# omarkhursheed/whisper-sae

Hardware: AMD Instinct MI355X
Metric: activations/sec through SAE train step (d=384->3072, k=32) (higher is better)
Workload: dtype bf16; 1 GPU; BASELINE.json configs[1]: TopKSAE 384->3072 k=32 train step, synthetic activations resident in the HBM ring buffer; batch_per_gpu=16384, global_batch=16384, ring_rows_per_gpu=4194304, parallelism=dp1

## Files before the change

include/wsae.h:

```cpp
#ifndef WSAE_H_
#define WSAE_H_

#include <stddef.h>
#include <stdint.h>

#ifdef __cplusplus
extern "C" {
#endif

#define WSAE_VERSION 1

#define WSAE_OK 0
#define WSAE_ERR_INVALID (-1)
#define WSAE_ERR_HIP (-2)
#define WSAE_ERR_NOMEM (-3)

#define WSAE_PREC_BF16 0
#define WSAE_PREC_FP32 1

#define WSAE_DT_F32 0
#define WSAE_DT_BF16 1

typedef struct wsae_ctx wsae_ctx;
typedef struct wsae_ring wsae_ring;

typedef struct wsae_config {
    int32_t input_dim;
    int32_t hidden_dim;
    int32_t k;
    int32_t max_batch;
    int32_t precision;
    int32_t device;
} wsae_config;

typedef struct wsae_stats {
    float loss;
    float l0;
    float grad_norm;
    float clip_coef;
    float dead_ratio;
    int32_t dead_count;
    int32_t topk_fallback_rows;
    int32_t reserved;
} wsae_stats;

const char* wsae_last_error(void);
int wsae_version(void);

int64_t wsae_param_count(int32_t input_dim, int32_t hidden_dim);
int wsae_param_offsets(int32_t input_dim, int32_t hidden_dim, int64_t offsets[5]);

int wsae_ctx_create(const wsae_config* cfg, wsae_ctx** out);
int wsae_ctx_destroy(wsae_ctx* ctx);
int wsae_ctx_set_fired(wsae_ctx* ctx, float* fired);
int wsae_ctx_set_strip_predict(wsae_ctx* ctx, int32_t on, float assume_store_threshold);
int wsae_ctx_strip_stats(wsae_ctx* ctx, int64_t* refilled_rows, float* last_min_threshold, float* margin);
int wsae_ctx_set_loss_cols(wsae_ctx* ctx, int32_t cols);
size_t wsae_ctx_workspace_bytes(const wsae_ctx* ctx);
int wsae_ctx_reserve_relu(wsae_ctx* ctx);

int wsae_prepare(wsae_ctx* ctx, const float* params, void* stream);


int wsae_encode_topk(wsae_ctx* ctx, const float* params, const void* x, int32_t x_dtype,
                     const int32_t* rows, int32_t B, float* vals, int32_t* idx,
                     int64_t* step_count, wsae_stats* stats, void* stream);

int wsae_encode_dense(wsae_ctx* ctx, const float* params, const void* x, int32_t x_dtype,
                      const int32_t* rows, int32_t B, float* pre, void* stream);

int wsae_densify(wsae_ctx* ctx, const float* vals, const int32_t* idx, int32_t B, float* hidden,
                 void* stream);

int wsae_decode_dense(wsae_ctx* ctx, const float* params, const float* hidden, int32_t B,
                      float* recon, void* stream);

int wsae_decode_loss(wsae_ctx* ctx, const float* params, const void* x, int32_t x_dtype,
                     const int32_t* rows, const float* vals, const int32_t* idx, int32_t B,
                     float* recon, int32_t want_bwd, float* dpre, int64_t* last_activated,
                     const int64_t* step_count, wsae_stats* stats, void* stream);

int wsae_encode_decode(wsae_ctx* ctx, const float* params, const void* x, int32_t x_dtype, const int32_t* rows,
                       int32_t B, float* vals, int32_t* idx, int64_t* step_count, float* recon, int32_t want_bwd,
                       float* dpre, int64_t* last_activated, wsae_stats* stats, void* stream);

int wsae_weight_grads(wsae_ctx* ctx, const float* params, const void* x, int32_t x_dtype,
                      const int32_t* rows, const float* vals, const int32_t* idx,
                      const float* dpre, int32_t B, float* grads, void* stream);

#define WSAE_BTK_TRAIN 0
#define WSAE_BTK_EVAL 1
#define WSAE_BTK_SELECT 2
typedef struct wsae_batch_topk_state {
    float threshold;
    float beta;
    float last_t;
    int32_t saturated_rows;
    int32_t kept;
    int32_t reserved[3];
} wsae_batch_topk_state;
int wsae_batch_topk_select(wsae_ctx* ctx, float* vals, int32_t B, int32_t k_batch, int32_t mode,
                           wsae_batch_topk_state* state, void* stream);
int wsae_ctx_set_batch_topk(wsae_ctx* ctx, int32_t k_batch, int32_t mode, wsae_batch_topk_state* state);

#define WSAE_PART_ALL (-1)
#define WSAE_PART_DECODER 0
#define WSAE_PART_ENCODER 1
int wsae_wgrad_parts_supported(const wsae_ctx* ctx);
int wsae_ctx_set_comm_reserve(wsae_ctx* ctx, int32_t n_cus);
int wsae_weight_grads_wire(wsae_ctx* ctx, const float* params, const void* x, int32_t x_dtype,
                           const int32_t* rows, const float* vals, const int32_t* idx, const float* dpre,
                           int32_t B, int32_t part, void* wire, int32_t wire_dtype, void* stream);

int wsae_last_residual_grad(wsae_ctx* ctx, int32_t B, float* g_out, void* stream);

int wsae_input_grad(wsae_ctx* ctx, const float* params, const int32_t* idx, const float* dpre,
                    int32_t B, float* dx, int32_t subtract_g, void* stream);

#define WSAE_WIRE_METRIC_SLOTS 24
int wsae_ctx_set_wire_metrics(wsae_ctx* ctx, const float* loss_l0);
int wsae_grads_unpack_wire(wsae_ctx* ctx, const void* wire, int32_t wire_dtype, float* grads_ext,
                           const float* metrics_sum, int32_t world, wsae_stats* stats, void* stream);
int wsae_adamw_step(wsae_ctx* ctx, float* params, const float* grads, float* exp_avg,
                    float* exp_avg_sq, float lr, float beta1, float beta2, float eps,
                    float weight_decay, int32_t step, float max_norm, float grad_scale,
                    int32_t normalize_decoder, int32_t norm_from_wgrad,
                    int64_t* last_activated, const int64_t* step_count,
                    int64_t dead_threshold, wsae_stats* stats, void* stream);

int wsae_normalize_decoder(wsae_ctx* ctx, float* params, void* stream);

int wsae_dead_scan(wsae_ctx* ctx, const int64_t* last_activated, const int64_t* step_count,
                   int64_t threshold, uint8_t* mask, wsae_stats* stats, void* stream);

int wsae_row_errors(wsae_ctx* ctx, const void* x, int32_t x_dtype, const int32_t* rows,
                    const float* recon, int32_t B, float* row_err, float* resid, void* stream);
int wsae_resample_dead(wsae_ctx* ctx, float* params, const void* inputs, int32_t x_dtype,
                       const int32_t* rows, int32_t Br, const float* row_err,
                       const uint8_t* dead_mask, int64_t* last_activated,
                       const int64_t* step_count, int32_t num_cap, int32_t* n_dead_out,
                       const float* dec_src, void* stream);

int wsae_ring_create(int32_t device, int64_t capacity_rows, int32_t dim, int32_t dtype,
                     wsae_ring** out);
int wsae_ring_destroy(wsae_ring* ring);
int wsae_ring_push_layernorm(wsae_ring* ring, const void* src, int32_t src_dtype, int64_t n_rows,
                             const float* gamma, const float* beta, float eps, void* stream);
void* wsae_ring_data(wsae_ring* ring);
int64_t wsae_ring_size(const wsae_ring* ring);
int wsae_ring_push(wsae_ring* ring, const void* src, int32_t src_dtype, int64_t n_rows, void* stream);
int wsae_ring_sample(wsae_ring* ring, uint64_t seed, int64_t epoch, int64_t offset, int32_t n,
                     int32_t* rows_out, void* stream);
int wsae_ring_fill_synthetic(wsae_ring* ring, uint64_t seed, int64_t n_rows, void* stream);

#define WSAE_IV_KEEP_ERROR 0
#define WSAE_IV_REPLACE 1
#define WSAE_IV_MAX_FORCE 64
int wsae_layernorm_rows(const void* src, int32_t src_dtype, int64_t n_rows, int32_t dim, const float* gamma,
                        const float* beta, float eps, void* dst, int32_t dst_dtype, void* stream);
int wsae_intervene(wsae_ctx* ctx, const float* params, const void* h, int32_t h_dtype, int64_t n_rows,
                   const float* vals, const int32_t* idx, const float* gamma, const float* beta, float eps,
                   const float* scale, const int32_t* force_idx, const float* force_val, int32_t n_force,
                   const uint8_t* row_mask, int32_t mode, void* out, int32_t out_dtype, int32_t* changed_rows,
                   void* stream);

#define WSAE_K_STAGE_BATCH 0
#define WSAE_K_ENCODE_GEMM 1
#define WSAE_K_TOPK 2
#define WSAE_K_DECODE 3
#define WSAE_K_BUCKET 4
#define WSAE_K_WGRAD 5
#define WSAE_K_WGRAD_REDUCE 6
#define WSAE_K_SQNORM 7
#define WSAE_K_ADAMW 8
#define WSAE_K_ROWNORM 9
#define WSAE_K_PREPARE 10
#define WSAE_K_DEAD_SCAN 11
#define WSAE_K_COUNT 12
const char* wsae_kernel_name(int32_t kernel_id);
int wsae_profile_enable(wsae_ctx* ctx, int32_t kernel_id, int32_t max_samples);
int wsae_profile_disable(wsae_ctx* ctx);
int wsae_profile_read(wsae_ctx* ctx, int32_t kernel_id, int32_t* n_launches, double* total_ms);

int64_t wsae_feature_topk_workspace_bytes(int64_t max_entries, int32_t H);
int wsae_feature_topk_update(const float* vals, const int32_t* idx, int64_t rows, int32_t width, int32_t H,
                             int32_t keep, int64_t ord_base, float* top_vals, int64_t* top_ord,
                             int32_t* top_cnt, int64_t* total_active, void* workspace,
                             int64_t workspace_bytes, void* stream);

int wsae_ctx_set_relu_fp8(wsae_ctx* ctx, int32_t on);
int wsae_relu_needs_hidden(const wsae_ctx* ctx, int32_t B);
int wsae_ctx_set_relu_l1_weights(wsae_ctx* ctx, const float* weights);
int wsae_relu_forward(wsae_ctx* ctx, const float* params, const void* x, int32_t x_dtype,
                      const int32_t* rows, int32_t B, float sparsity_weight, float* hidden,
                      float* recon, wsae_stats* stats, float* sparsity_loss_out, void* stream);
int wsae_relu_backward(wsae_ctx* ctx, const float* params, const void* x, int32_t x_dtype,
                       const int32_t* rows, int32_t B, float sparsity_weight, const float* hidden,
                       const float* recon, float* grads, void* stream);

#ifdef __cplusplus
}
#endif
#endif
```

whisper-sae_amd/csrc/wsae_ctx.hip:

```cpp
#include <stdarg.h>
#include <stdlib.h>
#include <string.h>

#include <new>

#include "wsae_common.h"
#include "wsae_topk.h"
#include <cstdlib>
#include <vector>

static thread_local char g_err[512] = "";
static void prof_free(wsae_ctx* c);

void wsae_set_error(const char* fmt, ...) {
    va_list ap;
    va_start(ap, fmt);
    vsnprintf(g_err, sizeof(g_err), fmt, ap);
    va_end(ap);
}

extern "C" const char* wsae_last_error(void) { return g_err; }
extern "C" int wsae_version(void) { return WSAE_VERSION; }

extern "C" int64_t wsae_param_count(int32_t D, int32_t H) {
// ... 111 lines not shown
    c->WdT_bf16 = (bf16_t*)(base + o_wd);
    c->c_fold = (float*)(base + o_cf);
    c->xb = base + o_xb;
    c->xT = base + o_xT;
    c->gT = base + o_gT;
    c->g = (float*)(base + o_g);
    c->gb = (bf16_t*)(base + o_gb);
    c->pre = (float*)(base + o_pre);
    c->smax = (float*)(base + o_sm);
    c->part_loss = (float*)(base + o_pl);
    c->part_l0 = (float*)(base + o_p0);
    c->part_dbd = (float*)(base + o_pd);
    c->part_sq = (float*)(base + o_ps);
    c->dbd2 = (float*)(base + o_d2);
    c->colnorm = (float*)(base + o_cn);
    c->counters = (int32_t*)(base + o_ct);
    c->wg_slabs = (float*)(base + o_ws);
    c->dbe_slab = (float*)(base + o_ds);
    c->dbpre_part = (float*)(base + o_dp);
    c->ent_pos = (uint32_t*)(base + o_ep);
    c->ent_hid = base + o_eh;
    c->ent_dpre = base + o_ed;
    c->ent_off = (int32_t*)(base + o_eo);
    c->dead_list = (int32_t*)(base + o_dl);
    c->row_order = (int32_t*)(base + o_ro);
    c->tmin = (uint32_t*)(base + o_tm);
    c->btk_ws = (int32_t*)(base + o_bt);
    const char* sp = getenv("WSAE_STRIP_PREDICT");
    c->strip_predict = (sp && sp[0] == '0') ? 0 : 1;
    const char* ss = getenv("WSAE_STRIP_SAFETY");
    c->tg_fixed_s = ss ? (float)atof(ss) : 0.f;
    c->ws_bytes = cv.total;
    *out = c;
    return WSAE_OK;
}

extern "C" int wsae_ctx_destroy(wsae_ctx* ctx) {
    if (!ctx) return WSAE_OK;
    prof_free(ctx);
    if (ctx->relu_ws) (void)hipFree(ctx->relu_ws);
    if (ctx->We_bf16) (void)hipFree((void*)ctx->We_bf16);
    delete ctx;
    return WSAE_OK;
}

static const char* const k_names[WSAE_K_COUNT] = {"stage_batch", "encode_gemm", "topk", "decode", "bucket", "wgrad",
                                                  "wgrad_reduce", "sqnorm", "adamw", "rownorm", "prepare", "dead_scan"};

extern "C" const char* wsae_kernel_name(int32_t id) { return (id >= 0 && id < WSAE_K_COUNT) ? k_names[id] : "?"; }

static void prof_free(wsae_ctx* c) {
    for (int k = 0; k < WSAE_K_COUNT; ++k) {
        if (c->prof.ev[k]) {
            for (int i = 0; i < 2 * c->prof.max_samples; ++i) (void)hipEventDestroy(c->prof.ev[k][i]);
            delete[] c->prof.ev[k];
            c->prof.ev[k] = nullptr;
        }
        c->prof.count[k] = 0;
    }
    c->prof.mask = 0;
    c->prof.max_samples = 0;
}

extern "C" int wsae_profile_disable(wsae_ctx* ctx) {
    WSAE_REQUIRE(ctx, "wsae_profile_disable: null ctx");
    prof_free(ctx);
    return WSAE_OK;
}

extern "C" int wsae_profile_enable(wsae_ctx* ctx, int32_t kernel_id, int32_t max_samples) {
    WSAE_REQUIRE(ctx && kernel_id >= -1 && kernel_id < WSAE_K_COUNT && max_samples >= 1 && max_samples <= 65536,
                 "wsae_profile_enable: bad argument");
    prof_free(ctx);
    ctx->prof.max_samples = max_samples;
    for (int k = 0; k < WSAE_K_COUNT; ++k) {
        if (kernel_id != -1 && kernel_id != k) continue;
        ctx->prof.ev[k] = new (std::nothrow) hipEvent_t[2 * (size_t)max_samples];
        if (!ctx->prof.ev[k]) {
            wsae_set_error("out of host memory");
            return WSAE_ERR_NOMEM;
        }
        for (int i = 0; i < 2 * max_samples; ++i) WSAE_HIP_CHECK(hipEventCreate(&ctx->prof.ev[k][i]));
        ctx->prof.mask |= 1u << k;
    }
    return WSAE_OK;
}

extern "C" int wsae_profile_read(wsae_ctx* ctx, int32_t kernel_id, int32_t* n_launches, double* total_ms) {
    WSAE_REQUIRE(ctx && kernel_id >= 0 && kernel_id < WSAE_K_COUNT && n_launches && total_ms,
                 "wsae_profile_read: bad argument");
    *n_launches = 0;
    *total_ms = 0.0;
    if (!ctx->prof.ev[kernel_id]) return WSAE_OK;
    const int n = ctx->prof.count[kernel_id];
    double tot = 0.0;
    for (int i = 0; i < n; ++i) {
        WSAE_HIP_CHECK(hipEventSynchronize(ctx->prof.ev[kernel_id][2 * i + 1]));
        float ms = 0.f;
        WSAE_HIP_CHECK(hipEventElapsedTime(&ms, ctx->prof.ev[kernel_id][2 * i], ctx->prof.ev[kernel_id][2 * i + 1]));
        tot += ms;
    }
    *n_launches = n;
    *total_ms = tot;
    return WSAE_OK;
}

extern "C" int wsae_ctx_set_fired(wsae_ctx* ctx, float* fired) {
    WSAE_REQUIRE(ctx, "wsae_ctx_set_fired: null ctx");
    ctx->fired = fired;
    return WSAE_OK;
}

static uint32_t host_f32_ord(float f) {
    uint32_t u;
    memcpy(&u, &f, 4);
    return (u & 0x80000000u) ? ~u : (u | 0x80000000u);
}
extern "C" int wsae_ctx_set_strip_predict(wsae_ctx* ctx, int32_t on, float assume_store_threshold) {
    WSAE_REQUIRE(ctx, "wsae_ctx_set_strip_predict: null ctx");
    ctx->strip_predict = on ? 1 : 0;
    ctx->pred_valid = 0;
    WSAE_HIP_CHECK(hipDeviceSynchronize());
    const bool forget = assume_store_threshold != assume_store_threshold;
    const float one = 1.0f;
    uint32_t hdr[3] = {forget ? 0u : host_f32_ord(assume_store_threshold), 0u, 0u};
    if (!forget) memcpy(&hdr[1], &one, 4);
    uint32_t* prev = ctx->tmin + ctx->tmin_cur * TG_GROUP_WORDS;
    WSAE_HIP_CHECK(hipMemset(prev, 0, TG_GROUP_WORDS * 4));
    WSAE_HIP_CHECK(hipMemset(ctx->tmin + ((ctx->tmin_cur + 2) % 3) * TG_GROUP_WORDS, 0, TG_GROUP_WORDS * 4));
    WSAE_HIP_CHECK(hipMemcpy(prev, hdr, sizeof(hdr), hipMemcpyHostToDevice));
    return WSAE_OK;
}
extern "C" int wsae_ctx_strip_stats(wsae_ctx* ctx, int64_t* refilled_rows, float* last_min_threshold, float* margin) {
    WSAE_REQUIRE(ctx && refilled_rows && last_min_threshold && margin, "wsae_ctx_strip_stats: null argument");
    std::vector<uint32_t> h(TG_WORDS);
    WSAE_HIP_CHECK(hipDeviceSynchronize());
    WSAE_HIP_CHECK(hipMemcpy(h.data(), ctx->tmin, h.size() * 4, hipMemcpyDeviceToHost));
    *refilled_rows = (int64_t)h[TG_REFILLED];
    uint32_t o = 0xFFFFFFFFu;
    for (int i = 0; i < TG_SLOTS; ++i) {
        const uint32_t s = h[ctx->tmin_cur * TG_GROUP_WORDS + i * TG_SLOT_STRIDE];
        if (s != 0u && s < o) o = s;
    }
    float f = NAN;
    if (o != 0u && o != 0xFFFFFFFFu) {
        const uint32_t u = (o & 0x80000000u) ? (o & 0x7FFFFFFFu) : ~o;
        memcpy(&f, &u, 4);
    }
    *last_min_threshold = f;
    memcpy(margin, &h[ctx->tmin_cur * TG_GROUP_WORDS + TG_HDR_S], 4);
    return WSAE_OK;
}

extern "C" int wsae_ctx_set_wire_metrics(wsae_ctx* ctx, const float* loss_l0) {
    WSAE_REQUIRE(ctx, "wsae_ctx_set_wire_metrics: null ctx");
    ctx->wire_metrics = loss_l0;
    return WSAE_OK;
}

extern "C" int wsae_ctx_set_loss_cols(wsae_ctx* ctx, int32_t cols) {
    WSAE_REQUIRE(ctx && cols >= 1 && cols <= ctx->D, "wsae_ctx_set_loss_cols: columns must be in [1, input_dim]");
    ctx->loss_cols = cols;
    return WSAE_OK;
}

extern "C" size_t wsae_ctx_workspace_bytes(const wsae_ctx* ctx) { return ctx ? ctx->ws_bytes : 0; }

__global__ void __launch_bounds__(256) prepare_kernel(const float* __restrict__ We, const float* __restrict__ WdT,
                                                      const float* __restrict__ be, const float* __restrict__ bpre,
                                                      bf16_t* __restrict__ We16, bf16_t* __restrict__ WdT16,
                                                      float* __restrict__ cfold, int H, int D) {
    const int lane = threadIdx.x & 63;
    const int h = blockIdx.x * 4 + (threadIdx.x >> 6);
    if (h >= H) return;
    const float* row = We + (int64_t)h * D;
    bf16_t* orow = We16 + (int64_t)h * D;
    const float* drow = WdT + (int64_t)h * D;
    bf16_t* odrow = WdT16 + (int64_t)h * D;
    float dot = 0.f;
    for (int d = lane * 4; d < D; d += 256) {
        const float4 wd = *(const float4*)(drow + d);
        bf16x4 o, e;
        o[0] = (bf16_t)wd.x; o[1] = (bf16_t)wd.y; o[2] = (bf16_t)wd.z; o[3] = (bf16_t)wd.w;
        *(bf16x4*)(odrow + d) = o;
        const float4 w = *(const float4*)(row + d);
        e[0] = (bf16_t)w.x; e[1] = (bf16_t)w.y; e[2] = (bf16_t)w.z; e[3] = (bf16_t)w.w;
        *(bf16x4*)(orow + d) = e;
        const float4 bp = *(const float4*)(bpre + d);
        dot = fmaf((float)e[0], bp.x, dot);
        dot = fmaf((float)e[1], bp.y, dot);
        dot = fmaf((float)e[2], bp.z, dot);
        dot = fmaf((float)e[3], bp.w, dot);
    }
    dot = wave_sum(dot);
    if (lane == 0) cfold[h] = be[h] - dot;
}

int wsae_prepare_launch(wsae_ctx* ctx, const float* params, hipStream_t st) {
    if (ctx->prec != WSAE_PREC_BF16) return WSAE_OK;
    WSAE_PROF_BEGIN(ctx, WSAE_K_PREPARE, st);
    prepare_kernel<<<ceil_div(ctx->H, 4), 256, 0, st>>>(params + ctx->off[0], params + ctx->off[1],
                                                        params + ctx->off[2], params + ctx->off[4], ctx->We_bf16,
                                                        ctx->WdT_bf16, ctx->c_fold, ctx->H, ctx->D);
    WSAE_PROF_END(ctx, WSAE_K_PREPARE, st);
    WSAE_LAUNCH_CHECK();
    return WSAE_OK;
}

extern "C" int wsae_prepare(wsae_ctx* ctx, const float* params, void* stream) {
    WSAE_REQUIRE(ctx && params, "wsae_prepare: null argument");
    return wsae_prepare_launch(ctx, params, (hipStream_t)stream);
}
```

whisper-sae_amd/csrc/wsae_encode.hip:

```cpp
#include "wsae_common.h"
#include "wsae_mfma.h"
#include "wsae_topk.h"

template <typename T>
__device__ __forceinline__ void store4(T* p, const float (&v)[4]) {
    if (sizeof(T) == 2) {
        bf16x4 o;
#pragma unroll
        for (int i = 0; i < 4; ++i) o[i] = (bf16_t)v[i];
        *(bf16x4*)p = o;
    } else {
        *(float4*)p = make_float4(v[0], v[1], v[2], v[3]);
    }
}

template <int XDT>
__device__ __forceinline__ void load4(const void* x, int64_t i, float (&v)[4]) {
    if (XDT == WSAE_DT_BF16) {
        const bf16x4 t = *(const bf16x4*)((const bf16_t*)x + i);
#pragma unroll
        for (int q = 0; q < 4; ++q) v[q] = (float)t[q];
    } else {
        const float4 t = *(const float4*)((const float*)x + i);
        v[0] = t.x; v[1] = t.y; v[2] = t.z; v[3] = t.w;
    }
}

template <int XDT, typename T>
__global__ void __launch_bounds__(256) stage_batch_kernel(const void* __restrict__ x, const int32_t* __restrict__ rows,
                                                          const float* __restrict__ bpre, T* __restrict__ xb,
                                                          T* __restrict__ xT, int B, int D, int ldT,
                                                          int64_t* __restrict__ step_count) {
    __shared__ float tile[64][65];
    if (step_count && blockIdx.x == 0 && blockIdx.y == 0 && threadIdx.x == 0) *step_count += 1;
    const int b0 = blockIdx.x * 64, d0 = blockIdx.y * 64;
    const int q = threadIdx.x & 15, r16 = threadIdx.x >> 4;
#pragma unroll
    for (int p = 0; p < 4; ++p) {
        const int bl = r16 + 16 * p, b = b0 + bl, d = d0 + 4 * q;
        float v[4] = {0.f, 0.f, 0.f, 0.f};
        if (b < B && d < D) {
            const int64_t src = rows ? (int64_t)rows[b] : (int64_t)b;
            load4<XDT>(x, src * D + d, v);
            if (sizeof(T) == 4) {
                const float4 bp = *(const float4*)(bpre + d);
                v[0] -= bp.x; v[1] -= bp.y; v[2] -= bp.z; v[3] -= bp.w;
            }
            store4<T>(xb + (int64_t)b * D + d, v);
        }
#pragma unroll
        for (int i = 0; i < 4; ++i) tile[bl][4 * q + i] = v[i];
    }
    if (!xT) return;
    __syncthreads();
#pragma unroll
    for (int p = 0; p < 4; ++p) {
        const int dl = r16 + 16 * p, d = d0 + dl, b = b0 + 4 * q;
        if (d < D && b < ldT) {
            float v[4];
#pragma unroll
            for (int i = 0; i < 4; ++i) v[i] = (T)tile[4 * q + i][dl];
            store4<T>(xT + (int64_t)d * ldT + b, v);
        }
    }
}

__global__ void __launch_bounds__(256) stage_rows_copy_kernel(const uint4* __restrict__ x, const int32_t* __restrict__ rows,
                                                              uint4* __restrict__ xb, int64_t nchunks, int cpr,
                                                              int64_t* __restrict__ step_count) {
    if (step_count && blockIdx.x == 0 && threadIdx.x == 0) *step_count += 1;
    const int64_t i0 = (int64_t)blockIdx.x * 512 + threadIdx.x, i1 = i0 + 256;
    const int64_t j0 = min(i0, nchunks - 1), j1 = min(i1, nchunks - 1);
    const int b0 = (int)(j0 / cpr), b1 = (int)(j1 / cpr);
    const int64_t r0 = rows ? (int64_t)rows[b0] : (int64_t)b0, r1 = rows ? (int64_t)rows[b1] : (int64_t)b1;
    const uint4 v0 = x[r0 * cpr + (j0 - (int64_t)b0 * cpr)];
    const uint4 v1 = x[r1 * cpr + (j1 - (int64_t)b1 * cpr)];
    if (i0 < nchunks) xb[i0] = v0;
    if (i1 < nchunks) xb[i1] = v1;
}

#ifdef WSAE_ENC_STAMPS
__device__ unsigned long long enc_stamp_sum[8];
#define EN_T(i)                                                                                     \
    {                                                                                               \
        __builtin_amdgcn_sched_barrier(0);                                                          \
        unsigned long long t_;                                                                      \
        asm volatile("s_memtime %0\n\ts_waitcnt lgkmcnt(0)" : "=s"(t_)::"memory");                  \
        __builtin_amdgcn_sched_barrier(0);                                                          \
        en_acc[i] += t_ - en_last;                                                                  \
        en_last = t_;                                                                               \
    }
extern "C" int wsae_debug_enc_stamps(double* out, int reset) {
    unsigned long long h[8];
    if (hipMemcpyFromSymbol(h, HIP_SYMBOL(enc_stamp_sum), sizeof(h)) != hipSuccess) return -1;
    for (int i = 0; i < 8; ++i) out[i] = (double)h[i];
    if (reset) {
        unsigned long long z[8] = {0, 0, 0, 0, 0, 0, 0, 0};
        (void)hipMemcpyToSymbol(HIP_SYMBOL(enc_stamp_sum), z, sizeof(z));
    }
    return 0;
}
#else
#define EN_T(i)
#endif
#define G256D_STAGE (2 * 256 * SWZ_ROW_BYTES)
#define G256D_STAGE1 (72 * 1024)
#define G256D_LDS (G256D_STAGE1 + G256D_STAGE)

template <typename T>
__global__ void __launch_bounds__(512)
encode_gemm256d_kernel(const T* __restrict__ xb, int64_t lda, const T* __restrict__ W, int64_t ldb,
                       const float* __restrict__ bias, float* __restrict__ pre, int64_t ldp, int B, int H, int D, int ntn,
                       int ntiles_mn, int nsplit, int64_t cz, float* __restrict__ smax, const int32_t* __restrict__ arows,
                       int64_t* __restrict__ step_count, const float* __restrict__ rscale = nullptr,
                       const float* __restrict__ cscale = nullptr, uint32_t* __restrict__ tmin = nullptr, int tmin_cur = 0,
                       float tg_fixed_s = 0.f) {
    extern __shared__ __attribute__((aligned(16))) char smem[];
    constexpr int KT = SWZ_ROW_BYTES / (int)sizeof(T);
    constexpr int EPC = 16 / (int)sizeof(T);
    const int tid = threadIdx.x, lane = tid & 63, wave = tid >> 6;
    const int wm = wave >> 2, wn = wave & 3;
    const int nk = D / KT;
    const int col = lane & 31, rq = lane >> 5;
    constexpr int PS = 68;
    float* patch = (float*)smem + wave * 32 * PS;
    const int pr = lane >> 4, pc = (lane & 15) * 4;
    const uint32_t smem_lds = (uint32_t)(uintptr_t)(__attribute__((address_space(3))) char*)smem;
    const int dma_r = lane >> 3, dma_s = lane & 7;
    if (step_count && blockIdx.x == 0 && tid == 0) *step_count += 1;
    __shared__ float tg_sh;
    if (wave == 0) {
        float s_now = 0.f;
        const float t = tmin ? strip_store_threshold(tmin, tmin_cur, lane, tg_fixed_s, &s_now) : -INFINITY;
        if (lane == 0) tg_sh = t;
        if (tmin && blockIdx.x == 0) {
            uint32_t* grp = tmin + tmin_cur * TG_GROUP_WORDS;
            grp[lane * TG_SLOT_STRIDE] = 0xFFFFFFFFu;
            if (lane == 0) {
                grp[TG_HDR_S] = __float_as_uint(s_now);
                grp[TG_HDR_MISSES] = 0u;
                __builtin_nontemporal_store(t, (float*)tmin + TG_USED);
            }
        }
    }

    const int ntiles = ntiles_mn * nsplit;
    const int ntm = ntiles_mn / ntn;
    const bool xcd_walk = nsplit == 1 && (gridDim.x % 8 == 0) && (ntm % 8 == 0);
    const int xcd = blockIdx.x & 7, local = blockIdx.x >> 3, per_xcd = gridDim.x >> 3;
    auto tile_at = [&](int i) -> int {
        if (!xcd_walk) return (int)blockIdx.x + i * (int)gridDim.x;
        const int tl = local + i * per_xcd;
        if (tl >= (ntm >> 3) * ntn) return ntiles;
        return (xcd * (ntm >> 3) + tl / ntn) * ntn + tl % ntn;
    };
    auto a_rows = [&](int m0, int (&ar)[4]) {
#pragma unroll
        for (int j = 0; j < 4; ++j) {
            const int m = min(m0 + (wave + 8 * j) * 8 + dma_r, B - 1);
            ar[j] = arows ? arows[m] : m;
        }
    };
    auto dma = [&](const int (&ar)[4], int n0, int64_t k0, int st) {
        const uint32_t base = smem_lds + (st ? G256D_STAGE1 : 0);
#pragma unroll
        for (int j = 0; j < 8; ++j) {
            const int piece = wave + 8 * j;
            const int row = (piece & 31) * 8 + dma_r;
            const int c = dma_s ^ ((row >> 1) & 7);
            const T* src = j < 4 ? xb + (int64_t)ar[j & 3] * lda + k0 + c * EPC
                                 : W + (int64_t)min(n0 + row, H - 1) * ldb + k0 + c * EPC;
            glds16(src, base + piece * 1024);
        }
    };
    auto m_of = [&](int t) { return ((t % ntiles_mn) / ntn) * 256; };
    auto n_of = [&](int t) { return ((t % ntiles_mn) % ntn) * 256; };
    auto k_of = [&](int t) { return (int64_t)(t / ntiles_mn) * D; };

#ifdef WSAE_ENC_STAMPS
    unsigned long long en_acc[8] = {0, 0, 0, 0, 0, 0, 0, 0}, en_last = __builtin_amdgcn_s_memtime();
#endif
    int it = 0, st = 1;
    int tile = tile_at(0);
    int ar[4] = {0, 0, 0, 0}, ar_n[4];
    if (tile < ntiles) {
        a_rows(m_of(tile), ar);
        dma(ar, n_of(tile), k_of(tile), st);
    }
    for (; tile < ntiles; tile = tile_at(++it)) {
        const int m0 = m_of(tile), n0 = n_of(tile);
        const int64_t kbase = k_of(tile);
        const int z = tile / ntiles_mn;
        f32x16 acc[4][2];
#pragma unroll
        for (int i = 0; i < 4; ++i)
#pragma unroll
            for (int j = 0; j < 2; ++j)
#pragma unroll
                for (int r = 0; r < 16; ++r) acc[i][j][r] = 0.f;
        const int nt = min(tile_at(it + 1), ntiles - 1);
        a_rows(m_of(nt), ar_n);
        EN_T(0)
        for (int kt = 0; kt < nk; ++kt) {
            dma_wait();
            EN_T(1)
            __syncthreads();
            EN_T(2)
            if (kt + 1 < nk) dma(ar, n0, kbase + (int64_t)(kt + 1) * KT, st ^ 1);
            else dma(ar_n, n_of(nt), k_of(nt), st ^ 1);
            EN_T(3)
            const char* As = smem + (st ? G256D_STAGE1 : 0);
            Mfma256s<T>::slab(As, As + 256 * SWZ_ROW_BYTES, wm * 128, wn * 64, lane, acc);
            st ^= 1;
            EN_T(4)
        }
        __syncthreads();
        EN_T(5)
        const int hcol = n0 + wn * 64 + pc;
        float4 bv4 = make_float4(0.f, 0.f, 0.f, 0.f);
        if (bias && z == 0 && hcol < H) bv4 = *(const float4*)(bias + hcol);
        const float tg = tg_sh;
        const bool fast = !rscale && smax && z == 0 && m0 + 256 <= B && n0 + 256 <= H && (int64_t)B * ldp < (1ll << 29);
        if (fast) {
            typedef int i32x4 __attribute__((ext_vector_type(4)));
            const __amdgpu_buffer_rsrc_t r_pre = __builtin_amdgcn_make_buffer_rsrc(pre, 0, 0x7fffffff, 0x00020000);
            const __amdgpu_buffer_rsrc_t r_sm = __builtin_amdgcn_make_buffer_rsrc(smax, 0, 0x7fffffff, 0x00020000);
            const int hs = H >> 4;
            const int b_lane = m0 + wm * 128 + pr;
            const int off_pre = (int)(((int64_t)b_lane * ldp + hcol) * 4);
            const int off_sm = (b_lane * hs + (hcol >> 4)) * 4;
            const int row_pre = (int)ldp * 16, row_sm = hs * 16;
#pragma unroll
            for (int mi = 0; mi < 4; ++mi) {
#pragma unroll
                for (int ni = 0; ni < 2; ++ni)
#pragma unroll
                    for (int r = 0; r < 16; ++r)
                        patch[((r & 3) + 8 * (r >> 2) + 4 * rq) * PS + ni * 32 + col] = acc[mi][ni][r];
                __builtin_amdgcn_wave_barrier();
                EN_T(6)
#pragma unroll
                for (int i = 0; i < 8; i += 2) {
                    f32x4 va = *(const f32x4*)(patch + (pr + 4 * i) * PS + pc);
                    f32x4 vb = *(const f32x4*)(patch + (pr + 4 * i + 4) * PS + pc);
                    va.x += bv4.x; va.y += bv4.y; va.z += bv4.z; va.w += bv4.w;
                    vb.x += bv4.x; vb.y += bv4.y; vb.z += bv4.z; vb.w += bv4.w;
                    const int q = mi * 8 + i;
                    float ma, mb, ta, tb;
                    asm volatile(
                        "v_max3_f32 %0, %4, %5, %6\n\t"
                        "v_max3_f32 %1, %8, %9, %10\n\t"
                        "v_max_f32 %0, %0, %7\n\t"
                        "v_max_f32 %1, %1, %11\n\t"
                        "s_nop 0\n\t"
                        "v_max_f32_dpp %2, %0, %0 quad_perm:[1,0,3,2] row_mask:0xf bank_mask:0xf\n\t"
                        "v_max_f32_dpp %3, %1, %1 quad_perm:[1,0,3,2] row_mask:0xf bank_mask:0xf\n\t"
                        "s_nop 0\n\t"
                        "v_max_f32_dpp %0, %2, %2 quad_perm:[2,3,0,1] row_mask:0xf bank_mask:0xf\n\t"
                        "v_max_f32_dpp %1, %3, %3 quad_perm:[2,3,0,1] row_mask:0xf bank_mask:0xf"
                        : "=&v"(ma), "=&v"(mb), "=&v"(ta), "=&v"(tb)
                        : "v"(va.x), "v"(va.y), "v"(va.z), "v"(va.w), "v"(vb.x), "v"(vb.y), "v"(vb.z), "v"(vb.w));
                    __builtin_amdgcn_raw_buffer_store_b32(__builtin_bit_cast(int, ma), r_sm, off_sm, q * row_sm, 0);
                    __builtin_amdgcn_raw_buffer_store_b32(__builtin_bit_cast(int, mb), r_sm, off_sm, (q + 1) * row_sm, 0);
                    if (!(ma < tg)) __builtin_amdgcn_raw_buffer_store_b128(__builtin_bit_cast(i32x4, va), r_pre, off_pre, q * row_pre, 2);
                    if (!(mb < tg)) __builtin_amdgcn_raw_buffer_store_b128(__builtin_bit_cast(i32x4, vb), r_pre, off_pre, (q + 1) * row_pre, 2);
                }
                __builtin_amdgcn_wave_barrier();
                EN_T(7)
            }
        } else {
            float4 cs4 = make_float4(1.f, 1.f, 1.f, 1.f);
            if (cscale && hcol < H) cs4 = *(const float4*)(cscale + hcol);
            float* Cz = pre + (int64_t)z * cz;
#pragma unroll
            for (int mi = 0; mi < 4; ++mi) {
#pragma unroll
                for (int ni = 0; ni < 2; ++ni)
#pragma unroll
                    for (int r = 0; r < 16; ++r)
                        patch[((r & 3) + 8 * (r >> 2) + 4 * rq) * PS + ni * 32 + col] = acc[mi][ni][r];
                __builtin_amdgcn_wave_barrier();
#pragma unroll
                for (int i = 0; i < 8; ++i) {
                    const int rl = pr + 4 * i;
                    const int b = m0 + wm * 128 + mi * 32 + rl;
                    float4 v = *(const float4*)(patch + rl * PS + pc);
                    if (rscale) {
                        const float rs = rscale[min(b, B - 1)];
                        v.x *= rs * cs4.x; v.y *= rs * cs4.y; v.z *= rs * cs4.z; v.w *= rs * cs4.w;
                    }
                    v.x += bv4.x; v.y += bv4.y; v.z += bv4.z; v.w += bv4.w;
                    if (b < B && hcol < H) *(float4*)(Cz + (int64_t)b * ldp + hcol) = v;
                    if (smax) {
                        float m = fmaxf(fmaxf(v.x, v.y), fmaxf(v.z, v.w));
                        m = fmaxf(m, __int_as_float(__builtin_amdgcn_update_dpp(0, __float_as_int(m), 0xB1, 0xF, 0xF, false)));
                        m = fmaxf(m, __int_as_float(__builtin_amdgcn_update_dpp(0, __float_as_int(m), 0x4E, 0xF, 0xF, false)));
                        if ((lane & 3) == 0 && b < B && hcol < H) smax[(int64_t)b * (H >> 4) + (hcol >> 4)] = m;
                    }
                }
                __builtin_amdgcn_wave_barrier();
            }
        }
#pragma unroll
        for (int j = 0; j < 4; ++j) ar[j] = ar_n[j];
    }
    dma_wait();
#ifdef WSAE_ENC_STAMPS
    if (lane == 0)
        for (int i = 0; i < 8; ++i) atomicAdd(&enc_stamp_sum[i], en_acc[i]);
#endif
}
template <typename T>
__device__ __forceinline__ void slab_load_rows(SlabRegs<T>& r, const T* __restrict__ base, int64_t ld, const int32_t* __restrict__ arows,
                                               int row0, int n_rows, int k0, int k_total, int tid) {
    constexpr int EPC = 16 / (int)sizeof(T);
    auto chunk = [&](int c) -> uint4 {
        const int row = row0 + (c >> 3), k = k0 + (c & 7) * EPC;
        if (row < n_rows && k < k_total) return *(const uint4*)(base + (int64_t)arows[row] * ld + k);
        return make_uint4(0, 0, 0, 0);
    };
    r.v0 = chunk(tid); r.v1 = chunk(tid + 256); r.v2 = chunk(tid + 512); r.v3 = chunk(tid + 768);
}

template <typename T>
__global__ void __launch_bounds__(256)
encode_gemm_kernel(const T* __restrict__ xb, const T* __restrict__ W, const float* __restrict__ bias,
                   float* __restrict__ pre, int ldp, int B, int H, int D, const int32_t* __restrict__ arows,
                   int64_t* __restrict__ step_count) {
    extern __shared__ __attribute__((aligned(16))) char smem[];
    char* As = smem;
    char* Bs = smem + TILE_LDS_BYTES;
    const int tid = threadIdx.x, lane = tid & 63, wave = tid >> 6;
    const int wm = wave >> 1, wn = wave & 1;
    const int m0 = blockIdx.y * TILE_M, n0 = blockIdx.x * TILE_N;
    constexpr int KT = Mfma<T>::KT;
    if (step_count && blockIdx.x == 0 && blockIdx.y == 0 && tid == 0) *step_count += 1;

    f32x16 acc[2][2];
#pragma unroll
    for (int i = 0; i < 2; ++i)
#pragma unroll
        for (int j = 0; j < 2; ++j)
#pragma unroll
            for (int r = 0; r < 16; ++r) acc[i][j][r] = 0.f;

    SlabRegs<T> ra, rb;
    if (arows) slab_load_rows<T>(ra, xb, D, arows, m0, B, 0, D, tid);
    else slab_load<T>(ra, xb, D, m0, B, 0, D, tid);
    slab_load<T>(rb, W, D, n0, H, 0, D, tid);
    const int nk = (D + KT - 1) / KT;
    for (int kt = 0; kt < nk; ++kt) {
        slab_store<T>(ra, As, tid);
        slab_store<T>(rb, Bs, tid);
        __syncthreads();
        if (kt + 1 < nk) {
            if (arows) slab_load_rows<T>(ra, xb, D, arows, m0, B, (kt + 1) * KT, D, tid);
            else slab_load<T>(ra, xb, D, m0, B, (kt + 1) * KT, D, tid);
            slab_load<T>(rb, W, D, n0, H, (kt + 1) * KT, D, tid);
        }
        Mfma<T>::slab(As, Bs, wm * 64, wn * 64, lane, acc);
        __syncthreads();
    }
    const int col = lane & 31, rq = lane >> 5;
#pragma unroll
    for (int mi = 0; mi < 2; ++mi)
#pragma unroll
        for (int ni = 0; ni < 2; ++ni) {
            const int h = n0 + wn * 64 + ni * 32 + col;
            if (h >= H) continue;
            const float bv = bias[h];
#pragma unroll
            for (int r = 0; r < 16; ++r) {
                const int b = m0 + wm * 64 + mi * 32 + (r & 3) + 8 * (r >> 2) + 4 * rq;
                if (b < B) pre[(int64_t)b * ldp + h] = acc[mi][ni][r] + bv;
            }
        }
}

__global__ void __launch_bounds__(256)
encode_direct_kernel(const bf16_t* __restrict__ xa, const int32_t* __restrict__ arows, const bf16_t* __restrict__ W,
                     const float* __restrict__ bias, float* __restrict__ pre, int ldp, int B, int H, int D,
                     int64_t* __restrict__ step_count) {
    const int lane = threadIdx.x & 63, wave = threadIdx.x >> 6;
    if (step_count && blockIdx.x == 0 && blockIdx.y == 0 && threadIdx.x == 0) *step_count += 1;
    const int n0 = blockIdx.x * 32, m0 = blockIdx.y * 128 + wave * 32;
    if (m0 >= B) return;
    const int r = lane & 31, h = lane >> 5;
    const int mrow = min(m0 + r, B - 1);
    const int64_t arow = arows ? (int64_t)arows[mrow] : (int64_t)mrow;
    const bf16_t* ap = xa + arow * D + 8 * h;
    const bf16_t* bp = W + (int64_t)min(n0 + r, H - 1) * D + 8 * h;
    f32x16 acc;
#pragma unroll
    for (int i = 0; i < 16; ++i) acc[i] = 0.f;
    const int nk = D / 16;
    for (int k0 = 0; k0 < nk; k0 += 8) {
        bf16x8 a[8], b[8];
#pragma unroll
        for (int j = 0; j < 8; ++j) {
            const int kk = min(k0 + j, nk - 1);
            a[j] = *(const bf16x8*)(ap + 16 * kk);
            b[j] = *(const bf16x8*)(bp + 16 * kk);
        }
#pragma unroll
        for (int j = 0; j < 8; ++j)
            if (k0 + j < nk) acc = __builtin_amdgcn_mfma_f32_32x32x16_bf16(a[j], b[j], acc, 0, 0, 0);
    }
    const int n = n0 + r;
    if (n >= H) return;
    const float bv = bias[n];
#pragma unroll
    for (int i = 0; i < 16; ++i) {
        const int m = m0 + (i & 3) + 8 * (i >> 2) + 4 * h;
        if (m < B) pre[(int64_t)m * ldp + n] = acc[i] + bv;
    }
}

#define TOPK_CAP 256

__global__ void __launch_bounds__(256) topk_kernel(const float* __restrict__ pre, int B, int H, int K,
                                                   float* __restrict__ vals, int32_t* __restrict__ idx,
                                                   int32_t* __restrict__ fallback_rows) {
    __shared__ uint64_t lists[4][TOPK_CAP];
    const int lane = threadIdx.x & 63, wave = threadIdx.x >> 6;
    const int b = blockIdx.x * 4 + wave;
    if (b >= B) return;
    const float* row = pre + (int64_t)b * H;
    uint64_t* list = lists[wave];
    float* vrow = vals + (int64_t)b * K;
    int32_t* irow = idx + (int64_t)b * K;

    uint64_t kmin = 0;
    if (K <= 64) {
        float m = -INFINITY;
        bool any = false;
        for (int e = lane * 4; e < H; e += 256) {
            const float4 v = *(const float4*)(row + e);
            m = fmaxf(fmaxf(m, fmaxf(v.x, v.y)), fmaxf(v.z, v.w));
            any = true;
        }
        uint64_t mk[1] = {any ? ((uint64_t)f32_ord(m) << 32) : 0ull};
        wave_sort_desc<1>(mk, lane);
        const uint32_t thi = __shfl((uint32_t)(mk[0] >> 32), K - 1, 64);
        kmin = (uint64_t)thi << 32;
    }
    const int count = topk_compact<TOPK_CAP>(row, H, kmin, list, lane);
    if (count > TOPK_CAP || count < K) {
        topk_row_generic<TOPK_CAP>(row, H, K, list, lane, vrow, irow, fallback_rows);
        return;
    }
    topk_emit_any<TOPK_CAP>(list, count, K, lane, vrow, irow);
}

#define TOPK_STRIP 8

template <int VPL>
__global__ void __launch_bounds__(256)
topk_rows_kernel(const float* __restrict__ pre, int B, int H, int K, float* __restrict__ vals,
                 int32_t* __restrict__ idx, int32_t* __restrict__ fallback_rows) {
    __shared__ uint64_t lists[4][TOPK_CAP];
    __shared__ uint64_t strips[4][64 * TOPK_STRIP];
    const int lane = threadIdx.x & 63, wave = threadIdx.x >> 6;
// ... 302 lines not shown
```

whisper-sae_amd/whisper_sae/_native.py:

```python

from __future__ import annotations

import ctypes as C
import os
from pathlib import Path

LIB_NAME = "libwsae_hip.so"

PREC_BF16, PREC_FP32 = 0, 1
DT_F32, DT_BF16 = 0, 1
PART_ALL, PART_DECODER, PART_ENCODER = -1, 0, 1
BTK_TRAIN, BTK_EVAL, BTK_SELECT = 0, 1, 2
IV_KEEP_ERROR, IV_REPLACE, IV_MAX_FORCE = 0, 1, 64
BTK_STATE_WORDS = 8


class WsaeError(RuntimeError):
    """A call into libwsae_hip failed (or the library is not built)."""


class Config(C.Structure):
    _fields_ = [("input_dim", C.c_int32), ("hidden_dim", C.c_int32), ("k", C.c_int32),
                ("max_batch", C.c_int32), ("precision", C.c_int32), ("device", C.c_int32)]


class Stats(C.Structure):

    _fields_ = [("loss", C.c_float), ("l0", C.c_float), ("grad_norm", C.c_float), ("clip_coef", C.c_float),
                ("dead_ratio", C.c_float), ("dead_count", C.c_int32), ("topk_fallback_rows", C.c_int32),
                ("reserved", C.c_int32)]


STATS_WORDS = C.sizeof(Stats) // 4

_p = C.c_void_p
_i32, _i64, _f32 = C.c_int32, C.c_int64, C.c_float

SIGNATURES = {
    "wsae_last_error": (C.c_char_p, []),
    "wsae_version": (C.c_int, []),
    "wsae_param_count": (_i64, [_i32, _i32]),
    "wsae_param_offsets": (C.c_int, [_i32, _i32, C.POINTER(_i64)]),
    "wsae_ctx_create": (C.c_int, [C.POINTER(Config), C.POINTER(_p)]),
    "wsae_ctx_destroy": (C.c_int, [_p]),
    "wsae_ctx_workspace_bytes": (C.c_size_t, [_p]),
    "wsae_ctx_set_loss_cols": (C.c_int, [_p, _i32]),
    "wsae_ctx_reserve_relu": (C.c_int, [_p]),
    "wsae_ctx_set_relu_fp8": (C.c_int, [_p, _i32]),
    "wsae_ctx_set_relu_l1_weights": (C.c_int, [_p, _p]),
    "wsae_ctx_set_strip_predict": (C.c_int, [_p, _i32, C.c_float]),
    "wsae_ctx_strip_stats": (C.c_int, [_p, _p, _p, _p]),
    "wsae_ctx_set_fired": (C.c_int, [_p, _p]),
    "wsae_ctx_set_wire_metrics": (C.c_int, [_p, _p]),
    "wsae_prepare": (C.c_int, [_p, _p, _p]),
    "wsae_encode_topk": (C.c_int, [_p, _p, _p, _i32, _p, _i32, _p, _p, _p, _p, _p]),
    "wsae_encode_dense": (C.c_int, [_p, _p, _p, _i32, _p, _i32, _p, _p]),
    "wsae_densify": (C.c_int, [_p, _p, _p, _i32, _p, _p]),
    "wsae_decode_dense": (C.c_int, [_p, _p, _p, _i32, _p, _p]),
    "wsae_feature_topk_workspace_bytes": (_i64, [_i64, _i32]),
    "wsae_feature_topk_update": (C.c_int, [_p, _p, _i64, _i32, _i32, _i32, _i64, _p, _p, _p, _p, _p, _i64, _p]),
    "wsae_decode_loss": (C.c_int, [_p, _p, _p, _i32, _p, _p, _p, _i32, _p, _i32, _p, _p, _p, _p, _p]),
    "wsae_encode_decode": (C.c_int, [_p, _p, _p, _i32, _p, _i32, _p, _p, _p, _p, _i32, _p, _p, _p, _p]),
    "wsae_weight_grads": (C.c_int, [_p, _p, _p, _i32, _p, _p, _p, _p, _i32, _p, _p]),
    "wsae_last_residual_grad": (C.c_int, [_p, _i32, _p, _p]),
    "wsae_input_grad": (C.c_int, [_p, _p, _p, _p, _i32, _p, _i32, _p]),
    "wsae_wgrad_parts_supported": (C.c_int, [_p]),
    "wsae_ctx_set_comm_reserve": (C.c_int, [_p, _i32]),
    "wsae_weight_grads_wire": (C.c_int, [_p, _p, _p, _i32, _p, _p, _p, _p, _i32, _i32, _p, _i32, _p]),
    "wsae_grads_unpack_wire": (C.c_int, [_p, _p, _i32, _p, _p, _i32, _p, _p]),
    "wsae_adamw_step": (C.c_int, [_p, _p, _p, _p, _p, _f32, _f32, _f32, _f32, _f32, _i32, _f32, _f32, _i32, _i32,
                                  _p, _p, _i64, _p, _p]),
    "wsae_normalize_decoder": (C.c_int, [_p, _p, _p]),
    "wsae_dead_scan": (C.c_int, [_p, _p, _p, _i64, _p, _p, _p]),
    "wsae_row_errors": (C.c_int, [_p, _p, _i32, _p, _p, _i32, _p, _p, _p]),
    "wsae_resample_dead": (C.c_int, [_p, _p, _p, _i32, _p, _i32, _p, _p, _p, _p, _i32, _p, _p, _p]),
    "wsae_ring_create": (C.c_int, [_i32, _i64, _i32, _i32, C.POINTER(_p)]),
    "wsae_ring_destroy": (C.c_int, [_p]),
    "wsae_ring_data": (_p, [_p]),
    "wsae_ring_size": (_i64, [_p]),
    "wsae_ring_push": (C.c_int, [_p, _p, _i32, _i64, _p]),
    "wsae_ring_push_layernorm": (C.c_int, [_p, _p, _i32, _i64, _p, _p, _f32, _p]),
    "wsae_ring_sample": (C.c_int, [_p, C.c_uint64, _i64, _i64, _i32, _p, _p]),
    "wsae_ring_fill_synthetic": (C.c_int, [_p, C.c_uint64, _i64, _p]),
    "wsae_kernel_name": (C.c_char_p, [_i32]),
    "wsae_profile_enable": (C.c_int, [_p, _i32, _i32]),
    "wsae_profile_disable": (C.c_int, [_p]),
    "wsae_profile_read": (C.c_int, [_p, _i32, C.POINTER(_i32), C.POINTER(C.c_double)]),
    "wsae_batch_topk_select": (C.c_int, [_p, _p, _i32, _i32, _i32, _p, _p]),
    "wsae_ctx_set_batch_topk": (C.c_int, [_p, _i32, _i32, _p]),
    "wsae_layernorm_rows": (C.c_int, [_p, _i32, _i64, _i32, _p, _p, _f32, _p, _i32, _p]),
    "wsae_intervene": (C.c_int, [_p, _p, _p, _i32, _i64, _p, _p, _p, _p, _f32, _p, _p, _p, _i32, _p, _i32, _p, _i32, _p,
                                 _p]),
    "wsae_relu_needs_hidden": (C.c_int, [_p, _i32]),
    "wsae_relu_forward": (C.c_int, [_p, _p, _p, _i32, _p, _i32, _f32, _p, _p, _p, _p, _p]),
    "wsae_relu_backward": (C.c_int, [_p, _p, _p, _i32, _p, _i32, _f32, _p, _p, _p, _p]),
}

_lib = None


def library_path() -> Path:
    env = os.environ.get("WSAE_LIB")
    return Path(env) if env else Path(__file__).resolve().parent / LIB_NAME


def lib() -> C.CDLL:
    global _lib
    if _lib is not None:
        return _lib
    import torch
    path = library_path()
    if not path.exists():
        raise WsaeError(
            f"{path} not found: the HIP extension is not built.  This package has no CPU path; build the "
            f"library with `make -C whisper-sae_amd/csrc` (hipcc, gfx950) or __graft_entry__.build().")
    try:
        handle = C.CDLL(str(path))
    except OSError as exc:
        raise WsaeError(f"could not load {path}: {exc}") from exc
    for name, (res, args) in SIGNATURES.items():
        try:
            fn = getattr(handle, name)
        except AttributeError as exc:
            raise WsaeError(f"{path} does not export {name}: stale build?") from exc
        fn.restype = res
        fn.argtypes = args
    _lib = handle
    return handle


def last_error() -> str:
    msg = lib().wsae_last_error()
    return msg.decode("utf-8", "replace") if msg else ""


def check(rc: int, what: str = "") -> None:
    if rc != 0:
        raise WsaeError(f"{what or 'libwsae_hip call'} failed (code {rc}): {last_error()}")


def param_count(input_dim: int, hidden_dim: int) -> int:
    return int(lib().wsae_param_count(input_dim, hidden_dim))


def param_offsets(input_dim: int, hidden_dim: int) -> list:
    arr = (_i64 * 5)()
    check(lib().wsae_param_offsets(input_dim, hidden_dim, arr), "wsae_param_offsets")
    return [int(v) for v in arr]


def pack_layout(input_dim: int, hidden_dim: int) -> tuple:
    d, h = input_dim, hidden_dim
    off = [0, d * h, 2 * d * h, 2 * d * h + h, 2 * d * h + h + d]
    return 2 * d * h + h + 2 * d, off


KERNEL_COUNT = 12
K_WGRAD = 5


def profile_read(handle: int) -> dict:
    out = {}
    for k in range(KERNEL_COUNT):
        n, ms = _i32(0), C.c_double(0.0)
        check(lib().wsae_profile_read(handle, k, C.byref(n), C.byref(ms)), "wsae_profile_read")
        if n.value:
            out[lib().wsae_kernel_name(k).decode()] = (n.value, ms.value)
    return out


def ptr(t) -> int:
    return 0 if t is None else t.data_ptr()

WIRE_METRIC_SLOTS = 24
```

Measured before the change: 73.51 million activations/s.

## Batch strip-max stores through LDS and use branchless OOB buffer stores in encode epilogue

In the bf16 encoder epilogue, the per-row strip maxima are first written into the LDS patch and then stored to global memory as one 128-bit buffer store per lane, instead of many scalar 32-bit stores. The conditional pre-activation stores become unconditional buffer stores that point at an out-of-bounds offset when the strip max is below the threshold, so no branch is needed. This depends on buffer resources with real byte limits. The bias load is moved ahead of the K loop for bf16 so its latency is hidden, and patch rows are processed in larger batches. It also adds a debug API to read strips and extra timing stamp slots.

```diff
diff --git a/include/wsae.h b/include/wsae.h
--- a/include/wsae.h
+++ b/include/wsae.h
@@ -55,6 +55,7 @@
 int wsae_ctx_set_fired(wsae_ctx* ctx, float* fired);
 int wsae_ctx_set_strip_predict(wsae_ctx* ctx, int32_t on, float assume_store_threshold);
 int wsae_ctx_strip_stats(wsae_ctx* ctx, int64_t* refilled_rows, float* last_min_threshold, float* margin);
+int wsae_ctx_debug_strips(wsae_ctx* ctx, int32_t B, float* pre, float* strip_max, float* store_threshold);
 int wsae_ctx_set_loss_cols(wsae_ctx* ctx, int32_t cols);
 size_t wsae_ctx_workspace_bytes(const wsae_ctx* ctx);
 int wsae_ctx_reserve_relu(wsae_ctx* ctx);
diff --git a/whisper-sae_amd/csrc/wsae_ctx.hip b/whisper-sae_amd/csrc/wsae_ctx.hip
--- a/whisper-sae_amd/csrc/wsae_ctx.hip
+++ b/whisper-sae_amd/csrc/wsae_ctx.hip
@@ -287,6 +287,19 @@
     return WSAE_OK;
 }
 
+extern "C" int wsae_ctx_debug_strips(wsae_ctx* ctx, int32_t B, float* pre, float* strip_max, float* store_threshold) {
+    WSAE_REQUIRE(ctx && B >= 1 && B <= ctx->maxB, "wsae_ctx_debug_strips: bad argument");
+    WSAE_REQUIRE(ctx->H % 16 == 0, "wsae_ctx_debug_strips: hidden_dim is not a multiple of 16");
+    WSAE_HIP_CHECK(hipDeviceSynchronize());
+    if (pre) WSAE_HIP_CHECK(hipMemcpy(pre, ctx->pre, (size_t)B * ctx->H * 4, hipMemcpyDefault));
+    if (strip_max) {
+        WSAE_REQUIRE(ctx->smax_valid, "wsae_ctx_debug_strips: the last encoder launch left no strip maxima");
+        WSAE_HIP_CHECK(hipMemcpy(strip_max, ctx->smax, (size_t)B * (ctx->H / 16) * 4, hipMemcpyDefault));
+    }
+    if (store_threshold) WSAE_HIP_CHECK(hipMemcpy(store_threshold, ctx->tmin + TG_USED, 4, hipMemcpyDefault));
+    return WSAE_OK;
+}
+
 extern "C" int wsae_ctx_set_wire_metrics(wsae_ctx* ctx, const float* loss_l0) {
     WSAE_REQUIRE(ctx, "wsae_ctx_set_wire_metrics: null ctx");
     ctx->wire_metrics = loss_l0;
diff --git a/whisper-sae_amd/csrc/wsae_encode.hip b/whisper-sae_amd/csrc/wsae_encode.hip
--- a/whisper-sae_amd/csrc/wsae_encode.hip
+++ b/whisper-sae_amd/csrc/wsae_encode.hip
@@ -80,7 +80,8 @@
 }
 
 #ifdef WSAE_ENC_STAMPS
-__device__ unsigned long long enc_stamp_sum[8];
+#define EN_STAMPS 10
+__device__ unsigned long long enc_stamp_sum[EN_STAMPS];
 #define EN_T(i)                                                                                     \
     {                                                                                               \
         __builtin_amdgcn_sched_barrier(0);                                                          \
@@ -91,11 +92,11 @@
         en_last = t_;                                                                               \
     }
 extern "C" int wsae_debug_enc_stamps(double* out, int reset) {
-    unsigned long long h[8];
+    unsigned long long h[EN_STAMPS];
     if (hipMemcpyFromSymbol(h, HIP_SYMBOL(enc_stamp_sum), sizeof(h)) != hipSuccess) return -1;
-    for (int i = 0; i < 8; ++i) out[i] = (double)h[i];
+    for (int i = 0; i < EN_STAMPS; ++i) out[i] = (double)h[i];
     if (reset) {
-        unsigned long long z[8] = {0, 0, 0, 0, 0, 0, 0, 0};
+        unsigned long long z[EN_STAMPS] = {};
         (void)hipMemcpyToSymbol(HIP_SYMBOL(enc_stamp_sum), z, sizeof(z));
     }
     return 0;
@@ -178,7 +179,7 @@
     auto k_of = [&](int t) { return (int64_t)(t / ntiles_mn) * D; };
 
 #ifdef WSAE_ENC_STAMPS
-    unsigned long long en_acc[8] = {0, 0, 0, 0, 0, 0, 0, 0}, en_last = __builtin_amdgcn_s_memtime();
+    unsigned long long en_acc[EN_STAMPS] = {}, en_last = __builtin_amdgcn_s_memtime();
 #endif
     int it = 0, st = 1;
     int tile = tile_at(0);
@@ -200,9 +201,15 @@
                 for (int r = 0; r < 16; ++r) acc[i][j][r] = 0.f;
         const int nt = min(tile_at(it + 1), ntiles - 1);
         a_rows(m_of(nt), ar_n);
+        constexpr bool BIAS_EARLY = sizeof(T) == 2;
+        const int hcol = n0 + wn * 64 + pc;
+        float4 bv4 = make_float4(0.f, 0.f, 0.f, 0.f);
+        if (BIAS_EARLY && bias && z == 0 && hcol < H) bv4 = *(const float4*)(bias + hcol);
         EN_T(0)
         for (int kt = 0; kt < nk; ++kt) {
             dma_wait();
+            if constexpr (BIAS_EARLY)
+                asm volatile("" : "+v"(bv4.x), "+v"(bv4.y), "+v"(bv4.z), "+v"(bv4.w));
             EN_T(1)
             __syncthreads();
             EN_T(2)
@@ -216,20 +223,21 @@
         }
         __syncthreads();
         EN_T(5)
-        const int hcol = n0 + wn * 64 + pc;
-        float4 bv4 = make_float4(0.f, 0.f, 0.f, 0.f);
-        if (bias && z == 0 && hcol < H) bv4 = *(const float4*)(bias + hcol);
+        if (!BIAS_EARLY && bias && z == 0 && hcol < H) bv4 = *(const float4*)(bias + hcol);
         const float tg = tg_sh;
         const bool fast = !rscale && smax && z == 0 && m0 + 256 <= B && n0 + 256 <= H && (int64_t)B * ldp < (1ll << 29);
         if (fast) {
             typedef int i32x4 __attribute__((ext_vector_type(4)));
-            const __amdgpu_buffer_rsrc_t r_pre = __builtin_amdgcn_make_buffer_rsrc(pre, 0, 0x7fffffff, 0x00020000);
-            const __amdgpu_buffer_rsrc_t r_sm = __builtin_amdgcn_make_buffer_rsrc(smax, 0, 0x7fffffff, 0x00020000);
+            constexpr int OOB_OFF = (int)0x80000000;
+            constexpr int RB = sizeof(T) == 2 ? 8 : 4;
             const int hs = H >> 4;
+            const __amdgpu_buffer_rsrc_t r_pre = __builtin_amdgcn_make_buffer_rsrc(pre, 0, (int)((int64_t)B * ldp * 4), 0x00020000);
+            const __amdgpu_buffer_rsrc_t r_sm = __builtin_amdgcn_make_buffer_rsrc(smax, 0, B * hs * 4, 0x00020000);
             const int b_lane = m0 + wm * 128 + pr;
             const int off_pre = (int)(((int64_t)b_lane * ldp + hcol) * 4);
-            const int off_sm = (b_lane * hs + (hcol >> 4)) * 4;
-            const int row_pre = (int)ldp * 16, row_sm = hs * 16;
+            const int row_pre = (int)ldp * 16;
+            const int off_sm = lane < 32 ? ((m0 + wm * 128 + lane) * hs + ((n0 + wn * 64) >> 4)) * 4 : OOB_OFF;
+            float* pmax = patch + pr * PS + 64 + (pc >> 4);
 #pragma unroll
             for (int mi = 0; mi < 4; ++mi) {
 #pragma unroll
@@ -240,33 +248,44 @@
                 __builtin_amdgcn_wave_barrier();
                 EN_T(6)
 #pragma unroll
-                for (int i = 0; i < 8; i += 2) {
-                    f32x4 va = *(const f32x4*)(patch + (pr + 4 * i) * PS + pc);
-                    f32x4 vb = *(const f32x4*)(patch + (pr + 4 * i + 4) * PS + pc);
-                    va.x += bv4.x; va.y += bv4.y; va.z += bv4.z; va.w += bv4.w;
-                    vb.x += bv4.x; vb.y += bv4.y; vb.z += bv4.z; vb.w += bv4.w;
-                    const int q = mi * 8 + i;
-                    float ma, mb, ta, tb;
-                    asm volatile(
-                        "v_max3_f32 %0, %4, %5, %6\n\t"
-                        "v_max3_f32 %1, %8, %9, %10\n\t"
-                        "v_max_f32 %0, %0, %7\n\t"
-                        "v_max_f32 %1, %1, %11\n\t"
-                        "s_nop 0\n\t"
-                        "v_max_f32_dpp %2, %0, %0 quad_perm:[1,0,3,2] row_mask:0xf bank_mask:0xf\n\t"
-                        "v_max_f32_dpp %3, %1, %1 quad_perm:[1,0,3,2] row_mask:0xf bank_mask:0xf\n\t"
-                        "s_nop 0\n\t"
-                        "v_max_f32_dpp %0, %2, %2 quad_perm:[2,3,0,1] row_mask:0xf bank_mask:0xf\n\t"
-                        "v_max_f32_dpp %1, %3, %3 quad_perm:[2,3,0,1] row_mask:0xf bank_mask:0xf"
-                        : "=&v"(ma), "=&v"(mb), "=&v"(ta), "=&v"(tb)
-                        : "v"(va.x), "v"(va.y), "v"(va.z), "v"(va.w), "v"(vb.x), "v"(vb.y), "v"(vb.z), "v"(vb.w));
-                    __builtin_amdgcn_raw_buffer_store_b32(__builtin_bit_cast(int, ma), r_sm, off_sm, q * row_sm, 0);
-                    __builtin_amdgcn_raw_buffer_store_b32(__builtin_bit_cast(int, mb), r_sm, off_sm, (q + 1) * row_sm, 0);
-                    if (!(ma < tg)) __builtin_amdgcn_raw_buffer_store_b128(__builtin_bit_cast(i32x4, va), r_pre, off_pre, q * row_pre, 2);
-                    if (!(mb < tg)) __builtin_amdgcn_raw_buffer_store_b128(__builtin_bit_cast(i32x4, vb), r_pre, off_pre, (q + 1) * row_pre, 2);
+                for (int i0 = 0; i0 < 8; i0 += RB) {
+                    f32x4 v[RB];
+#pragma unroll
+                    for (int i = 0; i < RB; ++i) v[i] = *(const f32x4*)(patch + (pr + 4 * (i0 + i)) * PS + pc);
+#pragma unroll
+                    for (int i = 0; i < RB; ++i) {
+                        v[i].x += bv4.x; v[i].y += bv4.y; v[i].z += bv4.z; v[i].w += bv4.w;
+                    }
+                    EN_T(7)
+#pragma unroll
+                    for (int i = i0; i < i0 + RB; i += 2) {
+                        const f32x4 va = v[i - i0], vb = v[i - i0 + 1];
+                        const int q = mi * 8 + i;
+                        float ma, mb, ta, tb;
+                        asm("v_max3_f32 %0, %4, %5, %6\n\t"
+                            "v_max3_f32 %1, %8, %9, %10\n\t"
+                            "v_max_f32 %0, %0, %7\n\t"
+                            "v_max_f32 %1, %1, %11\n\t"
+                            "s_nop 0\n\t"
+                            "v_max_f32_dpp %2, %0, %0 quad_perm:[1,0,3,2] row_mask:0xf bank_mask:0xf\n\t"
+                            "v_max_f32_dpp %3, %1, %1 quad_perm:[1,0,3,2] row_mask:0xf bank_mask:0xf\n\t"
+                            "s_nop 0\n\t"
+                            "v_max_f32_dpp %0, %2, %2 quad_perm:[2,3,0,1] row_mask:0xf bank_mask:0xf\n\t"
+                            "v_max_f32_dpp %1, %3, %3 quad_perm:[2,3,0,1] row_mask:0xf bank_mask:0xf"
+                            : "=&v"(ma), "=&v"(mb), "=&v"(ta), "=&v"(tb)
+                            : "v"(va.x), "v"(va.y), "v"(va.z), "v"(va.w), "v"(vb.x), "v"(vb.y), "v"(vb.z), "v"(vb.w));
+                        pmax[4 * i * PS] = ma;
+                        pmax[4 * (i + 1) * PS] = mb;
+                        __builtin_amdgcn_raw_buffer_store_b128(__builtin_bit_cast(i32x4, va), r_pre, ma < tg ? OOB_OFF : off_pre, q * row_pre, 2);
+                        __builtin_amdgcn_raw_buffer_store_b128(__builtin_bit_cast(i32x4, vb), r_pre, mb < tg ? OOB_OFF : off_pre, (q + 1) * row_pre, 2);
+                    }
                 }
                 __builtin_amdgcn_wave_barrier();
-                EN_T(7)
+                EN_T(8)
+                const f32x4 sm = *(const f32x4*)(patch + (lane & 31) * PS + 64);
+                __builtin_amdgcn_raw_buffer_store_b128(__builtin_bit_cast(i32x4, sm), r_sm, off_sm, mi * 32 * hs * 4, 0);
+                __builtin_amdgcn_wave_barrier();
+                EN_T(9)
             }
         } else {
             float4 cs4 = make_float4(1.f, 1.f, 1.f, 1.f);
@@ -307,7 +326,7 @@
     dma_wait();
 #ifdef WSAE_ENC_STAMPS
     if (lane == 0)
-        for (int i = 0; i < 8; ++i) atomicAdd(&enc_stamp_sum[i], en_acc[i]);
+        for (int i = 0; i < EN_STAMPS; ++i) atomicAdd(&enc_stamp_sum[i], en_acc[i]);
 #endif
 }
 template <typename T>
diff --git a/whisper-sae_amd/whisper_sae/_native.py b/whisper-sae_amd/whisper_sae/_native.py
--- a/whisper-sae_amd/whisper_sae/_native.py
+++ b/whisper-sae_amd/whisper_sae/_native.py
@@ -50,6 +50,7 @@
     "wsae_ctx_set_relu_l1_weights": (C.c_int, [_p, _p]),
     "wsae_ctx_set_strip_predict": (C.c_int, [_p, _i32, C.c_float]),
     "wsae_ctx_strip_stats": (C.c_int, [_p, _p, _p, _p]),
+    "wsae_ctx_debug_strips": (C.c_int, [_p, _i32, _p, _p, _p]),
     "wsae_ctx_set_fired": (C.c_int, [_p, _p]),
     "wsae_ctx_set_wire_metrics": (C.c_int, [_p, _p]),
     "wsae_prepare": (C.c_int, [_p, _p, _p]),
```

Result: no change. 73.45 million activations/s (-0.1%).
